# team-ergo-unipi/ergo_uvo

Measured on AMD Instinct MI355X. Metric: stereo frame-pairs/sec (detect+match+pose) @1920x1080, 3k kpts, higher is better.
Workload: dtype f32+f64

## Files before the change

ergo_uvo_amd/__init__.py:

```python
from __future__ import annotations

import collections
import ctypes as C

import numpy as np

from . import _lib

__all__ = ["Params", "Context", "StereoResult", "MonoResult", "UvoError", "KP_DTYPE", "DM_DTYPE", "build"]

build = _lib.build

KP_DTYPE = np.dtype([("x", "f4"), ("y", "f4"), ("size", "f4"), ("angle", "f4"), ("response", "f4"),
                     ("octave", "i4"), ("class_id", "i4")])
DM_DTYPE = np.dtype([("queryIdx", "i4"), ("trainIdx", "i4"), ("imgIdx", "i4"), ("distance", "f4")])

MEM_HOST, MEM_DEVICE = 0, 1
_STATUS = {1: "UVO_INVALID_ARG", 2: "UVO_TOO_FEW_POINTS", 3: "UVO_CAPACITY", 4: "UVO_HIP_ERROR", 5: "UVO_NO_DEVICE"}
_UVO_CAPACITY = 3


class UvoError(RuntimeError):
    def __init__(self, status: int, msg: str):
        super().__init__(f"{_STATUS.get(status, status)}: {msg}")
# ... 101 lines not shown
    def close(self):
        if getattr(self, "_h", None):
            self._lib.uvo_ctx_destroy(self._h)
            self._h = None

    def __del__(self):
        try:
            self.close()
        except Exception:
            pass

    @property
    def stream(self) -> int:
        return self._lib.uvo_ctx_stream(self._h)

    @property
    def warning(self) -> str:
        return (self._lib.uvo_ctx_warning(self._h) or b"").decode()

    def host_policy(self) -> dict:
        out = {}
        for kv in (self._lib.uvo_ctx_host_policy(self._h) or b"").decode().split():
            k, _, v = kv.partition("=")
            out[k] = float(v) if k == "cpu_budget" else (int(v) if k == "depth" else v)
        return out

    def set_producer_stream(self, stream):
        self._producer = stream
        if stream is None:
            self._check(self._lib.uvo_ctx_set_producer_stream(self._h, None, 0))
        elif stream != "torch":
            self._check(self._lib.uvo_ctx_set_producer_stream(self._h, C.c_void_p(int(getattr(stream, "cuda_stream", stream)) or None), 1))

    def _order_after_producer(self, *arrays):
        if self._producer == "torch" and any(_is_device(a) for a in arrays):
            import torch
            self._check(self._lib.uvo_ctx_set_producer_stream(self._h, C.c_void_p(torch.cuda.current_stream().cuda_stream or None), 1))

    def set_feature_detector(self, name: str):
        if name in ("AKAZE", "ORB"):
            self._check(self._lib.uvo_ctx_set_loop_detector(self._h, name.encode()))
            self._feature_akaze, self._feature_orb, self._feature_sift = name == "AKAZE", name == "ORB", False
            return
        self._check(self._lib.uvo_ctx_set_feature_detector(self._h, name.encode()))
        self._feature_sift = name == "SIFT"
        self._feature_akaze = self._feature_orb = False

# ... 473 lines not shown
```

ergo_uvo_amd/_lib.py:

```python
from __future__ import annotations

import ctypes as C
import os
import subprocess

_HERE = os.path.dirname(os.path.abspath(__file__))
CSRC = os.path.join(_HERE, "csrc")
LIB_PATH = os.environ.get("UVO_HIP_LIB") or os.path.join(_HERE, "lib", "libuvo_hip.so")

EXPORTS = [
    "uvo_params_default_stereo", "uvo_params_default_mono", "uvo_ctx_create", "uvo_ctx_destroy", "uvo_last_error",
    "uvo_ctx_stream", "uvo_ctx_set_params", "uvo_ctx_set_feature_detector", "uvo_ctx_set_loop_detector", "uvo_ctx_set_pnp_method", "uvo_ctx_set_producer_stream", "uvo_ctx_warning", "uvo_ctx_pending", "uvo_ctx_host_policy", "uvo_surf_detect", "uvo_sift_detect", "uvo_sift_layer", "uvo_akaze_detect", "uvo_akaze_plane", "uvo_orb_configure", "uvo_orb_set_pattern", "uvo_orb_detect", "uvo_orb_plane", "uvo_integral", "uvo_hessian_layer",
    "uvo_match_knn2_ratio", "uvo_match_knn2", "uvo_match_knn2_ratio_dim", "uvo_match_knn2_dim", "uvo_match_knn2_ratio_hamming", "uvo_match_knn2_hamming", "uvo_match_loop_knn2", "uvo_triangulate_points", "uvo_extract_3d_points",
    "uvo_solve_pnp_ransac", "uvo_reproject_errors", "uvo_rodrigues", "uvo_stereo_set_rig", "uvo_stereo_reset", "uvo_stereo_step",
    "uvo_stereo_set_depth", "uvo_stereo_submit", "uvo_stereo_collect",
    "uvo_stereo_get", "uvo_find_essential_mat", "uvo_recover_pose", "uvo_find_homography", "uvo_decompose_homography_mat",
    "uvo_recover_pose_homography", "uvo_select_estimation_method", "uvo_estimate_relative_pose", "uvo_mono_set_camera",
    "uvo_mono_reset", "uvo_mono_step", "uvo_mono_submit", "uvo_mono_collect", "uvo_mono_get", "uvo_get_image", "uvo_decode_image", "uvo_bayer_bggr2bgr", "uvo_resize_camera_matrix", "uvo_timing_enable", "uvo_timing_count", "uvo_timing_name", "uvo_timing_get", "uvo_timing_reset", "uvo_trace_enable", "uvo_trace_read",
]


EXPERIMENTAL = ["uvo_stereo_set_batch"]


def build(force: bool = False) -> str:
    srcs = [os.path.join(CSRC, f) for f in os.listdir(CSRC) if f.endswith((".hip", ".h"))]
    srcs.append(os.path.join(_HERE, "..", "include", "uvo_hip.h"))
    stale = not os.path.exists(LIB_PATH) or any(os.path.getmtime(s) > os.path.getmtime(LIB_PATH) for s in srcs)
    if force or stale:
        subprocess.check_call(["make", "-C", CSRC, "-s", "-j4"])
    return LIB_PATH


_lib = None


def lib() -> C.CDLL:
    global _lib
    if _lib is None:
        if not os.path.exists(LIB_PATH):
            build()
        try:
            import torch
        except ImportError:
            pass
# ... 3 lines not shown
        _lib.uvo_ctx_stream.restype = C.c_void_p
        _lib.uvo_ctx_stream.argtypes = [C.c_void_p]
        _lib.uvo_ctx_warning.restype = C.c_char_p
        _lib.uvo_ctx_warning.argtypes = [C.c_void_p]
        _lib.uvo_ctx_host_policy.restype = C.c_char_p
        _lib.uvo_ctx_host_policy.argtypes = [C.c_void_p]
        _lib.uvo_ctx_set_producer_stream.argtypes = [C.c_void_p, C.c_void_p, C.c_int]
        _lib.uvo_decode_image.argtypes = [C.c_void_p, C.c_void_p, C.c_size_t, C.c_char_p, C.c_void_p, C.c_size_t, C.c_int, C.c_void_p, C.c_void_p, C.c_void_p]
        _lib.uvo_sift_detect.argtypes = [C.c_void_p, C.c_void_p, C.c_int, C.c_int, C.c_int, C.c_int, C.c_int, C.c_int, C.c_double, C.c_double, C.c_double, C.c_void_p, C.c_void_p, C.c_int, C.c_void_p]
        _lib.uvo_ctx_set_feature_detector.argtypes = [C.c_void_p, C.c_char_p]
        _lib.uvo_ctx_set_loop_detector.argtypes = [C.c_void_p, C.c_char_p]
        _lib.uvo_ctx_set_pnp_method.argtypes = [C.c_void_p, C.c_int]
        _lib.uvo_match_loop_knn2.argtypes = [C.c_void_p, C.c_void_p, C.c_int, C.c_void_p, C.c_int, C.c_int, C.c_int, C.c_void_p, C.c_void_p]
        _lib.uvo_ctx_pending.restype = C.c_int
        _lib.uvo_ctx_pending.argtypes = [C.c_void_p]
        _lib.uvo_ctx_destroy.argtypes = [C.c_void_p]
        _lib.uvo_ctx_destroy.restype = None
        _lib.uvo_timing_name.restype = C.c_char_p
        _lib.uvo_timing_name.argtypes = [C.c_void_p, C.c_int]
        _lib.uvo_trace_read.restype = C.c_int
        _lib.uvo_trace_read.argtypes = [C.c_void_p, C.c_void_p, C.c_int]
        _lib.uvo_trace_enable.argtypes = [C.c_void_p, C.c_int]
        for name in EXPORTS + EXPERIMENTAL:
            getattr(_lib, name)
    return _lib
```

ergo_uvo_amd/csrc/ctx.hip:

```cpp
#include "uvo_ctx.h"
#include <pthread.h>
#include "uvo_epnp.h"
#include <string.h>
#include <sched.h>
#include <atomic>
#include <math.h>
#include <float.h>
#include <new>
#include <algorithm>
#include <atomic>
namespace uvo { extern bool g_bdbg; extern std::atomic<double> g_bstat[16]; double now_us(); void operator+=(std::atomic<double>& a, double v); }

using namespace uvo;

struct uvo_ctx : public uvo::Ctx {};

namespace {
uvo_status abi_caught(uvo_ctx* c) noexcept
{
    uvo_status st = UVO_HIP_ERROR;
    const char* what = "unexpected C++ exception inside libuvo_hip";
    static thread_local char text[160];
    try { throw; }
    catch (const std::bad_alloc&) { st = UVO_CAPACITY; what = "out of host memory (std::bad_alloc) inside libuvo_hip"; }
// ... 46 lines not shown

static void lane_worker(uvo_ctx* L);
__global__ void k_prime(int* sink, int n);
static void run_stage_b(uvo_ctx* L, bool stage_a_ok);
static uvo_status prime_lanes(uvo_ctx* c, int w, int h);
extern "C" uvo_status uvo_mono_collect(uvo_ctx* c, double dt, uvo_mono_result* out);
static void run_mono_stage_b(uvo_ctx* L, bool stage_a_ok);
static void destroy_one(uvo_ctx* c);
static uvo_status queue_stage_a(uvo_ctx* c, uvo_ctx* A, uvo_ctx* B);
struct GatherPair;
static hipError_t trace_alloc(Ctx* c)
{
    if (c->trace.empty()) {
        c->trace.resize(Ctx::kTraceRing);
        for (auto& r : c->trace) for (int k = 0; k < 8; k++) { hipError_t e = hipEventCreate(&r.ev[k]); if (e != hipSuccess) return e; }
    }
    c->trace_on = true;
    return hipSuccess;
}

namespace {
std::mutex g_pool_mu;
hipStream_t g_pool[64][2][uvo::Ctx::kMaxDepth];
bool pool_on() { static const bool on = !(getenv("UVO_STREAM_POOL") && atoi(getenv("UVO_STREAM_POOL")) == 0); return on; }
hipError_t stream_acquire(int device, int role, int lane, hipStream_t* out)
{
    if (pool_on() && lane >= 0 && lane < uvo::Ctx::kMaxDepth) {
        std::lock_guard<std::mutex> lk(g_pool_mu);
        hipStream_t& slot = g_pool[device & 63][role][lane];
        if (slot) { *out = slot; slot = nullptr; return hipSuccess; }
    }
    return hipStreamCreateWithFlags(out, hipStreamNonBlocking);
}
void stream_release(int device, int role, int lane, hipStream_t s)
{
    if (!s) return;
    (void)hipStreamSynchronize(s);
    if (pool_on() && lane >= 0 && lane < uvo::Ctx::kMaxDepth) {
        std::lock_guard<std::mutex> lk(g_pool_mu);
        hipStream_t& slot = g_pool[device & 63][role][lane];
        if (!slot) { slot = s; return; }
    }
    (void)hipStreamDestroy(s);
}
}

static const char* unsupported_params(const uvo_params* p)
{
    if (p->ITERATIONS_COUNT > 0 && p->PNP_METHOD_FLAG != 1)
        return "PNP_METHOD_FLAG: uvo_params takes only 1 (cv::SOLVEPNP_EPNP, the value shipped in stereo_VO_parameters.yaml); 2 (P3P), 3 (DLS) and 4 (UPNP) "
               "are set with uvo_ctx_set_pnp_method, 0 (ITERATIVE), 5 (AP3P) and above are not implemented";
    if (p->USE_EXTRINSIC_GUESS != 0) return "USE_EXTRINSIC_GUESS: only false is implemented (EPnP ignores the guess)";
    return nullptr;
}

static thread_local const char* t_create_refusal = nullptr;

static uvo_status create_one(const uvo_params* p, int device, int max_w, int max_h, int max_kpts, uvo_ctx** out, int lane = 0)
{
    if (!out) return UVO_INVALID_ARG;
    *out = nullptr;
    t_create_refusal = p ? unsupported_params(p) : nullptr;
    if (!p || max_w < 16 || max_h < 16 || max_kpts < 16 || t_create_refusal) return UVO_INVALID_ARG;
    int ndev = 0;
    if (hipGetDeviceCount(&ndev) != hipSuccess || ndev <= 0 || device < 0 || device >= ndev) return UVO_NO_DEVICE;
    if (hipSetDevice(device) != hipSuccess) return UVO_HIP_ERROR;
    uvo_ctx* c = new (std::nothrow) uvo_ctx();
    if (!c) return UVO_HIP_ERROR;
    c->p = *p; c->device = device; c->max_w = max_w; c->max_h = max_h; c->cap = max_kpts; c->lane_id = lane;
    const size_t cap = (size_t)max_kpts;
    const size_t npx = (size_t)max_w * max_h, nsum = (size_t)(max_w + 1) * (max_h + 1);
    const int nstrip = (max_h + 7) / 8;
    c->colpart_stride = ((max_w + 1 + 2047) / 2048) * 2048;
    const size_t nchunks = (cap + 127) / 128;
    hipError_t e = hipSuccess;
#define A(expr) do { if (e == hipSuccess) e = (expr); } while (0)
    A(stream_acquire(device, 0, lane, &c->stream));
    A(hipEventCreate(&c->ev0)); A(hipEventCreate(&c->ev1));
    c->plane_pw = ((max_w + 1 + 3) / 4 + 1 + 1) & ~1;
    c->plane_stride = c->plane_pw * ((max_h + 1 + 3) / 4 + 1);
    for (int i = 0; i < 2; i++) {
        A(dalloc(&c->d_planes[i], (size_t)16 * c->plane_stride));
        if (e == hipSuccess) e = hipMemset(c->d_planes[i], 0, sizeof(int32_t) * 16 * c->plane_stride);
        A(dalloc(&c->d_img[i], npx)); A(dalloc(&c->d_sum_base[i], nsum + 2 * kSumPad));
        if (e == hipSuccess) { e = hipMemset(c->d_sum_base[i], 0, sizeof(int32_t) * (nsum + 2 * kSumPad)); c->d_sum[i] = c->d_sum_base[i] + kSumPad; }
        A(dalloc(&c->d_cand[i], cap)); A(dalloc(&c->det[i].kps, cap)); A(dalloc(&c->det[i].desc, cap * 128));
        A(dalloc(&c->d_tmp_desc[i], cap * 128)); A(dalloc(&c->d_matches[i], cap));
        A(dalloc(&c->d_as_kpsL[i], cap)); A(dalloc(&c->d_as_kpsR[i], cap)); A(dalloc(&c->d_as_descL[i], cap * 128));
        A(dalloc(&c->d_as_pts4[i], cap)); A(dalloc(&c->d_as_cam1[i], cap * 3)); A(dalloc(&c->d_as_flag[i], cap));
    }
    c->surv_cap = 4 * (int)cap; A(dalloc(&c->d_surv, (size_t)c->surv_cap));
    A(dalloc(&c->d_colpart, (size_t)2 * nstrip * c->colpart_stride));
    A(dalloc(&c->d_DW, 400)); A(dalloc(&c->d_rank, cap * 2)); A(dalloc(&c->d_big_par, cap * 4)); A(dalloc(&c->d_big_patch, cap * 2 * 448));
    A(dalloc(&c->d_mpart, 2 * nchunks * cap)); A(dalloc(&c->d_mscratch, 2 * (nchunks + 4))); A(dalloc(&c->d_knn_idx, 2 * cap * 2)); A(dalloc(&c->d_knn_dist, 2 * cap * 2));
    A(dalloc(&c->d_x1, cap)); A(dalloc(&c->d_x2, cap)); A(dalloc(&c->d_xc, cap)); A(dalloc(&c->d_pts4, cap));
    A(dalloc(&c->d_cam1, cap * 3)); A(dalloc(&c->d_flag, cap)); A(dalloc(&c->d_tmp_idx, cap)); A(dalloc(&c->d_tmp_row, cap));
    if (const char* ww = getenv("UVO_WORKER_WAIT")) c->worker_wait = !strcmp(ww, "spin") ? 0 : (!strcmp(ww, "block-all") ? 2 : ((!strcmp(ww, "sleep") || !strcmp(ww, "block")) ? 3 : 1));
    c->wait_eff.store(c->worker_wait == 0 ? 0 : (c->worker_wait == 2 ? 2 : 1), std::memory_order_relaxed);
    A(hipEventCreateWithFlags(&c->evBlock, hipEventDisableTiming | hipEventBlockingSync));
    A(hipEventCreateWithFlags(&c->evPoll, hipEventDisableTiming));
    A(hipEventCreateWithFlags(&c->evB, hipEventDisableTiming | (c->worker_wait == 2 ? hipEventBlockingSync : 0)));
    for (int i = 0; i < 2; i++) {
        A(dalloc(&c->d_good_pts[i], cap * 3)); A(dalloc(&c->d_good_idx[i], cap));
        A(dalloc(&c->d_opts[i], cap * 3)); A(dalloc(&c->d_ipts[i], cap));
        A(hipEventCreateWithFlags(&c->evA[i], hipEventDisableTiming | ((i == 0 && c->worker_wait == 2) ? hipEventBlockingSync : 0)));
        A(hipHostMalloc(reinterpret_cast<void**>(&c->h_countsA[i]), sizeof(int) * CN_TOTAL));
    }
    A(hipEventCreateWithFlags(&c->evAS, hipEventDisableTiming));
    A(hipEventCreateWithFlags(&c->evSync, hipEventDisableTiming));
    A(hipEventCreateWithFlags(&c->evProducer, hipEventDisableTiming));
    A(hipEventCreateWithFlags(&c->evDet, hipEventDisableTiming)); A(hipEventCreateWithFlags(&c->evPrevRead, hipEventDisableTiming));
    {
        int least = 0, greatest = 0;
        const char* pe = getenv("UVO_PNP_PRIORITY");
        if (pe && atoi(pe) != 0 && hipDeviceGetStreamPriorityRange(&least, &greatest) == hipSuccess && greatest != least)
            A(hipStreamCreateWithPriority(&c->pnp_stream, hipStreamNonBlocking, greatest));
        else
            A(stream_acquire(device, 1, lane, &c->pnp_stream));
    }
    A(dalloc(&c->d_countsB, (size_t)4)); A(hipHostMalloc(reinterpret_cast<void**>(&c->h_countsB), sizeof(int) * 4));
    A(dalloc(&c->d_counts, (size_t)CN_TOTAL));
    A(dalloc(&c->d_subsets, (size_t)kMaxHyp * 5)); A(dalloc(&c->d_models, (size_t)kMaxHyp * 6)); A(dalloc(&c->d_hcount, (size_t)kMaxHyp));
    A(dalloc(&c->d_inliers, cap)); A(dalloc(&c->d_refit, cap * 21)); A(dalloc(&c->d_pose, (size_t)6));
    A(hipHostMalloc(reinterpret_cast<void**>(&c->h_counts), sizeof(int) * CN_TOTAL));
    A(hipHostMalloc(reinterpret_cast<void**>(&c->h_subsets), sizeof(int) * kMaxHyp * 5));
    A(hipHostMalloc(reinterpret_cast<void**>(&c->h_hcount), sizeof(int) * kMaxHyp));
    A(hipHostMalloc(reinterpret_cast<void**>(&c->h_pose), sizeof(double) * 6));
    A(dalloc(&c->d_rng_raw, (size_t)1024)); A(hipMalloc(&c->d_spec, 64)); A(hipHostMalloc(&c->h_spec, 64));
#undef A
    if (e != hipSuccess) { destroy_one(c); return UVO_HIP_ERROR; }
    c->d_cand_n = c->d_counts + CN_CAND0;
    c->det[0].n = c->d_counts + CN_NL; c->det[1].n = c->d_counts + CN_NR;
    c->d_nmatch = c->d_counts + CN_M;
    c->d_as_n = c->d_counts + CN_AS0;
    c->d_big_n = c->d_counts + CN_BIG0;
    if (surf_build_area_tables(c) != UVO_OK) { destroy_one(c); return UVO_HIP_ERROR; }
    {
        std::vector<unsigned> raw(1024);
        uint64_t state = (uint64_t)-1;
        for (auto& v : raw) v = rng_next(state);
        if (hipMemcpy(c->d_rng_raw, raw.data(), sizeof(unsigned) * raw.size(), hipMemcpyHostToDevice) != hipSuccess ||
// ... 48 lines not shown
        double q = -1, per = 0;
        if (FILE* g = fopen("/sys/fs/cgroup/cpu/cpu.cfs_quota_us", "r")) { if (fscanf(g, "%lf", &q) != 1) q = -1; fclose(g); }
        if (FILE* g = fopen("/sys/fs/cgroup/cpu/cpu.cfs_period_us", "r")) { if (fscanf(g, "%lf", &per) != 1) per = 0; fclose(g); }
        if (q > 0 && per > 0) b = std::min(b, q / per);
    }
    if (const char* e = getenv("UVO_CPU_BUDGET")) { const double v = atof(e); if (v > 0) b = std::min(b, v); }
    return b;
}
static void apply_wait_policy(uvo_ctx* c)
{
    const int depth = (int)c->lanes.size();
    c->cpu_budget = host_cpu_budget();
    int eff = c->worker_wait == 0 ? 0 : (c->worker_wait == 2 ? 2 : 1);
    if (c->worker_wait == 1 && c->cpu_budget >= 2.0 * (depth + 2)) eff = 0;
    for (Ctx* l : c->lanes) l->wait_eff.store(eff, std::memory_order_release);
    if (const char* e = getenv("UVO_STAGE_B")) c->stage_b_mode = !strcmp(e, "device") ? 1 : (!strcmp(e, "worker") ? 0 : -1);
}
static bool stage_b_on_device(const uvo_ctx* c)
{
    if (c->stage_b_mode >= 0) return c->stage_b_mode == 1;
    return c->cpu_budget < (double)c->lanes.size() + 3.0;
}

static uvo_status set_depth(uvo_ctx* c, int depth)
{
    if (depth < 1 || depth > Ctx::kMaxDepth) { c->err = "pipeline depth must be 1..16"; return UVO_INVALID_ARG; }
    if (c->n_pending != 0) { c->err = "pipeline depth cannot change while pairs are in flight"; return UVO_INVALID_ARG; }
    while ((int)c->lanes.size() > depth) { destroy_one(static_cast<uvo_ctx*>(c->lanes.back())); c->lanes.pop_back(); }
    while ((int)c->lanes.size() < depth) {
        uvo_ctx* l = nullptr;
        uvo_status st = create_one(&c->p, c->device, c->max_w, c->max_h, c->cap, &l, (int)c->lanes.size());
        if (st != UVO_OK) { c->err = "could not allocate a further pipeline lane"; return st; }
        l->master = c; l->lane_id = (int)c->lanes.size(); l->timing = c->timing;
        if (c->trace_on && !l->trace_on && trace_alloc(l) != hipSuccess) { destroy_one(l); c->err = "could not allocate a further pipeline lane"; return UVO_HIP_ERROR; }
        c->lanes.push_back(l);
    }
    apply_wait_policy(c);
    c->warning.clear();
    {
        const char* q = getenv("GPU_MAX_HW_QUEUES");
        const int nq = q ? atoi(q) : 4;
        if (depth > 2 && nq < 2 * depth)
            c->warning = "GPU_MAX_HW_QUEUES = " + std::to_string(nq) + " with " + std::to_string(depth) + " pipeline lanes (two HIP streams each): lanes share "
                         "hardware queues and the pipeline runs well below its rate; set GPU_MAX_HW_QUEUES >= " + std::to_string(2 * depth) + " before the HIP runtime starts";
    }
    if (c->primed_w > 0) UVO_TRY(prime_lanes(c, c->primed_w, c->primed_h));
    if (c->prev_lane >= depth || c->next_lane >= depth) { c->vo_initialized = false; c->init_matches.clear(); c->prev_lane = 0; c->next_lane = 0; c->prev_sync = true; }
    return UVO_OK;
}

static void precreate_streams(int device)
{
    static const int order = getenv("UVO_STREAM_ORDER") ? atoi(getenv("UVO_STREAM_ORDER")) : 0;
    if (order < 1 || order > 2 || !pool_on()) return;
    const int depth = getenv("UVO_PIPELINE_DEPTH") ? std::min((int)uvo::Ctx::kMaxDepth, std::max(1, atoi(getenv("UVO_PIPELINE_DEPTH")))) : 6;
    if (hipSetDevice(device) != hipSuccess) return;
    std::lock_guard<std::mutex> lk(g_pool_mu);
    int* sink = nullptr;
    if (hipMalloc(reinterpret_cast<void**>(&sink), 64) != hipSuccess) return;
    for (int pass = 0; pass < 2; pass++) {
        const int role = order == 1 ? pass : 1 - pass;
        for (int l = 0; l < depth; l++) {
            hipStream_t& slot = g_pool[device & 63][role][l];
            if (slot) continue;
            if (hipStreamCreateWithFlags(&slot, hipStreamNonBlocking) != hipSuccess) { slot = nullptr; continue; }
            hipLaunchKernelGGL(k_prime, dim3(1), dim3(64), 0, slot, sink, 1);
            (void)hipStreamSynchronize(slot);
        }
    }
    (void)hipFree(sink);
}

extern "C" uvo_status uvo_ctx_create(const uvo_params* p, int device, int max_w, int max_h, int max_kpts, uvo_ctx** out)
try {
    precreate_streams(device);
    uvo_status st = create_one(p, device, max_w, max_h, max_kpts, out);
    if (st != UVO_OK) return st;
    (*out)->lanes.push_back(*out);
    if (getenv("UVO_MAX_B")) (*out)->max_b = std::min(16, std::max(1, atoi(getenv("UVO_MAX_B"))));
    if (getenv("UVO_A_OVERLAP")) (*out)->a_overlap = std::min(16, std::max(0, atoi(getenv("UVO_A_OVERLAP"))));
    if (getenv("UVO_MAX_B_MONO")) (*out)->max_b_mono = std::min(16, std::max(1, atoi(getenv("UVO_MAX_B_MONO"))));
    if (getenv("UVO_A_OVERLAP2")) (*out)->a_overlap2 = std::min(4, std::max(0, atoi(getenv("UVO_A_OVERLAP2"))));
    if (getenv("UVO_BATCH")) (*out)->batch = atoi(getenv("UVO_BATCH")) == 2 ? 2 : 1;
    if (getenv("UVO_A_OVERLAP_MONO")) (*out)->a_overlap_mono = std::min(8, std::max(0, atoi(getenv("UVO_A_OVERLAP_MONO"))));
    st = set_depth(*out, 2);
    if (st != UVO_OK) { uvo_ctx_destroy(*out); *out = nullptr; }
    return st;
} UVO_ABI_CATCH(nullptr)

extern "C" uvo_status uvo_stereo_set_batch(uvo_ctx* c, int pairs)
try {
    if (!c) return UVO_INVALID_ARG;
    if (pairs != 1 && pairs != 2) { c->err = "uvo_stereo_set_batch: 1 or 2 pairs per launch set"; return UVO_INVALID_ARG; }
    if (c->n_pending != 0) { c->err = "the launch mode cannot change while pairs are in flight"; return UVO_INVALID_ARG; }
    c->batch = pairs;
    return UVO_OK;
} UVO_ABI_CATCH(c)

// ... 33 lines not shown
    }
    if (c->stream) (void)hipStreamSynchronize(c->stream);
    for (int i = 0; i < 2; i++) {
        (void)hipFree(c->d_img[i]); (void)hipFree(c->d_sum_base[i]); (void)hipFree(c->d_planes[i]); (void)hipFree(c->d_cand[i]); (void)hipFree(c->det[i].kps);
        (void)hipFree(c->det[i].desc); (void)hipFree(c->d_tmp_desc[i]); (void)hipFree(c->d_matches[i]);
        (void)hipFree(c->d_as_kpsL[i]); (void)hipFree(c->d_as_kpsR[i]); (void)hipFree(c->d_as_descL[i]);
        (void)hipFree(c->d_as_pts4[i]); (void)hipFree(c->d_as_cam1[i]); (void)hipFree(c->d_as_flag[i]);
    }
    if (c->pnp_stream) (void)hipStreamSynchronize(c->pnp_stream);
    mono_ws_free(c);
    pre_ws_free(c);
    codec_ws_free(c);
    sift_ws_free(c);
    akaze_ws_free(c);
    orb_ws_free(c);
    void* ptrs[] = { c->d_hess_order, c->d_surv, c->d_octpat, c->d_colpart, c->d_DW, c->d_rank, c->d_big_par, c->d_big_patch, c->d_area_tabs, c->d_area_iscale, c->d_ori_w, c->d_mpart, c->d_mscratch, c->d_knn_idx, c->d_knn_dist, c->d_x1, c->d_x2, c->d_xc, c->d_pts4, c->d_cam1,
                     c->d_flag, c->d_tmp_idx, c->d_tmp_row, c->d_good_pts[0], c->d_good_pts[1], c->d_good_idx[0], c->d_good_idx[1], c->d_opts[0], c->d_opts[1],
                     c->d_ipts[0], c->d_ipts[1], c->d_counts, c->d_countsB, c->d_subsets, c->d_models,
                     c->d_hcount, c->d_inliers, c->d_refit, c->d_pose };
    for (void* p : ptrs) (void)hipFree(p);
    (void)hipHostFree(c->h_counts); (void)hipHostFree(c->h_subsets); (void)hipHostFree(c->h_hcount); (void)hipHostFree(c->h_pose);
    (void)hipHostFree(c->h_countsB); (void)hipHostFree(c->h_spec); (void)hipFree(c->d_rng_raw); (void)hipFree(c->d_spec);
    for (int i = 0; i < 2; i++) { (void)hipHostFree(c->h_countsA[i]); if (c->evA[i]) (void)hipEventDestroy(c->evA[i]); }
    {
        const char* pe = getenv("UVO_PNP_PRIORITY");
        if (c->pnp_stream && pe && atoi(pe) != 0) (void)hipStreamDestroy(c->pnp_stream);
        else stream_release(c->device, 1, c->lane_id, c->pnp_stream);
    }
    if (c->evAS) (void)hipEventDestroy(c->evAS);
    if (c->evBlock) (void)hipEventDestroy(c->evBlock);
    if (c->evPoll) (void)hipEventDestroy(c->evPoll);
    if (c->evB) (void)hipEventDestroy(c->evB);
    if (c->evSync) (void)hipEventDestroy(c->evSync);
    if (c->evProducer) (void)hipEventDestroy(c->evProducer);
    for (auto& r : c->trace) for (int k = 0; k < 8; k++) if (r.ev[k]) (void)hipEventDestroy(r.ev[k]);
    if (c->evDet) (void)hipEventDestroy(c->evDet);
    if (c->evPrevRead) (void)hipEventDestroy(c->evPrevRead);
    if (c->ev0) (void)hipEventDestroy(c->ev0);
    if (c->ev1) (void)hipEventDestroy(c->ev1);
    stream_release(c->device, 0, c->lane_id, c->stream);
    delete c;
}

extern "C" const char* uvo_last_error(const uvo_ctx* c) { return c ? c->err.c_str() : (t_create_refusal ? t_create_refusal : "null context"); }
extern "C" void* uvo_ctx_stream(uvo_ctx* c) { return c ? (void*)c->stream : nullptr; }
extern "C" uvo_status uvo_ctx_set_params(uvo_ctx* c, const uvo_params* p)
try {
    if (!c || !p) return UVO_INVALID_ARG;
    if (c->n_pending != 0) { c->err = "parameters cannot change while pairs are in flight"; return UVO_INVALID_ARG; }
    if (const char* why = unsupported_params(p)) { c->err = why; return UVO_INVALID_ARG; }
    if ((p->SURF_EXTENDED != 0) != (c->p.SURF_EXTENDED != 0) && (c->vo_initialized || c->mono_initialized)) {
        c->err = "SURF_EXTENDED changes the descriptor width: the previous frame's descriptors held by the running VO loop would not match (uvo_stereo_reset / uvo_mono_reset first)";
        return UVO_INVALID_ARG;
    }
    for (Ctx* l : c->lanes) l->p = *p;
    return UVO_OK;
} UVO_ABI_CATCH(c)
extern "C" uvo_status uvo_ctx_set_producer_stream(uvo_ctx* c, void* hip_stream, int enabled)
try {
    if (!c) return UVO_INVALID_ARG;
    c->producer_stream = static_cast<hipStream_t>(hip_stream); c->has_producer = enabled != 0;
    return UVO_OK;
} UVO_ABI_CATCH(c)
extern "C" const char* uvo_ctx_warning(const uvo_ctx* c) { return c ? c->warning.c_str() : ""; }
extern "C" int uvo_ctx_pending(const uvo_ctx* c) { return c ? c->n_pending : 0; }
extern "C" const char* uvo_ctx_host_policy(uvo_ctx* c)
try {
    if (!c) return "";
    static const char* const wn[3] = { "poll", "timed-sleep+poll", "interrupt" };
    char buf[160];
    snprintf(buf, sizeof(buf), "wait=%s stage_b=%s cpu_budget=%.2f depth=%d", wn[c->wait_eff.load() % 3], stage_b_on_device(c) ? "device" : "worker",
             c->cpu_budget > 1e8 ? -1.0 : c->cpu_budget, (int)c->lanes.size());
    c->policy_text = buf;
    return c->policy_text.c_str();
} UVO_ABI_CATCH_RET(c, "")

static uvo_status wait_for_producer(uvo_ctx* m, Ctx* L, int mem)
{
    if (mem != UVO_MEM_DEVICE || !m->has_producer) return UVO_OK;
    UVO_HIP_TRY(m, hipEventRecord(L->evProducer, m->producer_stream));
    UVO_HIP_TRY(m, hipStreamWaitEvent(L->stream, L->evProducer, 0));
    return UVO_OK;
}
static uvo_status need_idle(uvo_ctx* c, const char* who)
{
    if (c->n_pending == 0) return UVO_OK;
    c->err = std::string(who) + ": collect the pairs / frames in flight first (the operator uses lane 0's buffers)";
    return UVO_INVALID_ARG;
}

static uvo_status fail(uvo_ctx* c, uvo_status s, const char* msg) { c->err = msg; return s; }

namespace uvo {
static inline void poll_pause() { for (int i = 0; i < 40; i++) __builtin_ia32_pause(); }
hipError_t poll_event(hipEvent_t ev)
// ... 643 lines not shown
    const int depth = (int)c->lanes.size();
    if (c->n_pending >= depth) return fail(c, UVO_INVALID_ARG, "uvo_stereo_submit: the pipeline is full; collect a pair first (uvo_stereo_set_depth)");
    if (c->timing && c->n_pending > 0) return fail(c, UVO_INVALID_ARG, "timing mode measures one pair at a time: collect before submitting");
    (void)hipSetDevice(c->device);
    const uvo_params& p = c->p;
    if (!c->vo_initialized) {
        uvo_stereo_result res;
        memset(&res, 0, sizeof(res));
        UVO_TRY(wait_for_producer(c, c, mem));
        UVO_TRY(surf_upload(c, 0, left, w, h, stride, mem));
        UVO_TRY(surf_upload(c, 1, right, w, h, stride, mem));
        UVO_TRY(detect_dispatch(c, 2));
        UVO_TRY(stereo_init_step(c, &res));
        UVO_TRY(prime_lanes(c, w, h));
        UVO_TRY(prepare_lane_detectors(c, w, h, 2));
        c->stereo_init_results.push_back(res);
        c->inflight[c->n_pending++] = Ctx::kInflightStereoInit; c->n_submitted++;
        c->next_lane = 0;
        return UVO_OK;
    }
    const int li = c->next_lane;
    Range r_submit("uvo:stereo_submit");
    uvo_ctx* L = static_cast<uvo_ctx*>(c->lanes[li]);
    L->pending = Ctx::Pending();
    L->pending.used = true;
    Ctx::StagePlan& pl = L->plan;
    pl.lane = li; pl.prev_lane = c->prev_lane; pl.prev_buf = c->prev_buf; pl.prev_sync = c->prev_sync; pl.curr = L->as_w;
    pl.pending_before = c->n_pending; pl.trace_slot = -1;
    if (L->trace_on) {
        L->trace_cur = (int)(L->trace_count++ % Ctx::kTraceRing);
        pl.trace_slot = L->trace_cur;
        Ctx::TraceRec* tr = &L->trace[L->trace_cur];
        tr->pair = c->n_submitted; tr->b_used = false; tr->det_marked = false;
        for (double& v : tr->host_us) v = 0;
        tr->host_us[0] = uvo::now_us();
    }
    const bool may_batch = c->batch == 2 && depth >= 2 && !c->in_sync_step && !c->timing && c->loop_detector() == 0 && p.SURF_UPRIGHT && p.SURF_OCTAVES_NUMBER == 4;
    uvo_ctx* S = c->stashed_lane >= 0 ? static_cast<uvo_ctx*>(c->lanes[c->stashed_lane]) : nullptr;
    hipStream_t own = L->stream;
    if (S && may_batch) L->stream = S->stream;
    uvo_status up = wait_for_producer(c, L, mem);
    if (up == UVO_OK) up = surf_upload(L, 0, left, w, h, stride, mem);
    if (up == UVO_OK) up = surf_upload(L, 1, right, w, h, stride, mem);
    L->stream = own;
    if (up != UVO_OK) { if (L != c) c->err = L->err; L->pending.used = false; return up; }
    L->as_w = pl.curr ^ 1;
// ... 186 lines not shown
static void lane_worker(uvo_ctx* L)
{
    { char nm[16]; snprintf(nm, sizeof(nm), "uvo-lane%d", L->lane_id); (void)pthread_setname_np(pthread_self(), nm); }
    (void)hipSetDevice(L->device);
    std::unique_lock<std::mutex> lk(L->mu);
    for (;;) {
        if (L->job.state != 1 && !L->quit) { lk.unlock(); poll_job_state(L, 1, 2000.0); lk.lock(); }
        L->cv.wait(lk, [&] { return L->quit || L->job.state == 1; });
        if (L->quit) return;
        lk.unlock();
        const double t0 = g_bdbg ? now_us() : 0;
        const bool stage_a_ok = wait_stage_a(L);
        if (g_bdbg) g_bstat[0] += now_us() - t0;
        Ctx::TraceRec* wtr = (L->trace_on && L->trace_cur >= 0 && L->job.kind == 0) ? &L->trace[L->trace_cur] : nullptr;
        if (wtr) wtr->host_us[3] = now_us();
        {
            Ctx* m = L->master ? L->master : L;
            std::unique_lock<std::mutex> g(m->b_mu);
            const double tw = g_bdbg ? now_us() : 0;
            const int limit = L->job.kind == 1 ? m->max_b_mono : m->max_b;
            m->b_cv.wait(g, [&] { return m->b_running < limit; });
            if (g_bdbg) g_bstat[5] += now_us() - tw;
            m->b_running++;
            g.unlock();
            if (wtr) wtr->host_us[4] = now_us();
            try {
                if (L->job.kind == 1) { const double tb = g_bdbg ? now_us() : 0; run_mono_stage_b(L, stage_a_ok); if (g_bdbg) { g_bstat[1] += now_us() - tb; g_bstat[4] += 1; } }
                else if (L->job.kind == 2) { hipLaunchKernelGGL(k_prime, dim3(1), dim3(64), 0, L->pnp_stream, L->d_countsB, 1); (void)host_sync(L, L->pnp_stream); }
                else run_stage_b(L, stage_a_ok);
            } catch (...) {
                L->job.st = abi_caught(L); L->job.ran = 0;
                try { L->job.err = L->err; } catch (...) { L->job.err.clear(); }
            }
            if (wtr) wtr->host_us[5] = now_us();
            g.lock();
            m->b_running--;
            m->b_cv.notify_one();
        }
        lk.lock();
        L->job.state = 2;
        L->job_state_a.store(2, std::memory_order_release);
        L->cv.notify_all();
    }
}

extern "C" uvo_status uvo_stereo_collect(uvo_ctx* c, double dt, uvo_stereo_result* out)
try {
    if (!c || !out) return UVO_INVALID_ARG;
    if (c->n_pending <= 0) return fail(c, UVO_INVALID_ARG, "uvo_stereo_collect: nothing submitted");
    if (c->inflight[0] == Ctx::kInflightMonoInit || (c->inflight[0] >= 0 && c->lanes[c->inflight[0]]->job.kind != 0))
        return fail(c, UVO_INVALID_ARG, "uvo_stereo_collect: the oldest entry in flight is a mono frame (uvo_mono_collect)");
    (void)hipSetDevice(c->device);
    Range r_collect("uvo:stereo_collect");
    const uvo_params& p = c->p;
    const int li = c->inflight[0];
    for (int i = 1; i < c->n_pending; i++) c->inflight[i - 1] = c->inflight[i];
    c->n_pending--; c->n_collected++;
    if (li == Ctx::kInflightStereoInit) {
// ... 499 lines not shown
    if (c->mono_matched) {
        if (c->use_binary()) UVO_TRY(match_knn2_bin(c, BIN_L2, reinterpret_cast<const uint8_t*>(c->d_as_descL[0]), nullptr, c->mono_n_prev,
                                                    reinterpret_cast<const uint8_t*>(c->det[0].desc), c->det[0].n, c->cap));
        else UVO_TRY(match_knn2(c, c->d_as_descL[0], nullptr, c->mono_n_prev, c->det[0].desc, c->det[0].n, c->cap));
        UVO_TRY(match_ratio_compact(c, nullptr, c->mono_n_prev, (float)p.LOWE_RATIO_THRESHOLD, c->d_matches[0], c->d_nmatch, c->cap));
        hipLaunchKernelGGL(k_gather_mono_pairs, dim3((c->cap + 255) / 256), dim3(256), 0, c->stream, c->d_matches[0], c->d_counts + CN_M, c->cap,
                           c->d_as_kpsL[0], c->det[0].kps, c->d_x1, c->d_x2);
        UVO_HIP_TRY(c, hipGetLastError());
        UVO_TRY(mono_prep_launch(c, c->stream, c->mono_K, p.DISTANCE));
    }
    UVO_HIP_TRY(c, hipMemcpyAsync(c->h_countsA[0], c->d_counts, sizeof(int) * CN_TOTAL, hipMemcpyDeviceToHost, c->stream));
    UVO_HIP_TRY(c, host_sync(c, c->stream));
    memcpy(c->h_counts, c->h_countsA[0], sizeof(int) * CN_TOTAL);
    UVO_TRY(check_cand_overflow(c, 1));
    const int n = c->h_counts[CN_NL];
    out->n_kps = n;
    c->kp_hint = n;
    c->mono_dev_n = n;
    auto roll_state = [&]() -> uvo_status {
        if (n) {
            UVO_HIP_TRY(c, hipMemcpyAsync(c->d_as_descL[0], c->det[0].desc, sizeof(float) * c->loop_words() * (size_t)n, hipMemcpyDeviceToDevice, c->stream));
            UVO_HIP_TRY(c, hipMemcpyAsync(c->d_as_kpsL[0], c->det[0].kps, sizeof(uvo_keypoint) * (size_t)n, hipMemcpyDeviceToDevice, c->stream));
        }
        c->mono_n_prev = n;
        return UVO_OK;
    };
    if (!c->mono_initialized) {
        UVO_TRY(roll_state());
        if (n >= p.MIN_NUM_FEATURES) c->mono_initialized = true;
        return UVO_OK;
    }
    c->job.kind = 1; c->job.range = range;
    run_mono_stage_b(c, true);
    if (c->job.st != UVO_OK) { const uvo_status st_ = c->job.st; c->err = c->job.err; return st_; }
    apply_mono_result(c, c->job, dt, out);
    return roll_state();
} UVO_ABI_CATCH(c)

extern "C" uvo_status uvo_mono_submit(uvo_ctx* c, const uint8_t* img, int w, int h, int stride, int mem, double range)
try {
    if (!c || !img) return UVO_INVALID_ARG;
    if (!c->mono_cam_set) return fail(c, UVO_INVALID_ARG, "uvo_mono_set_camera has not been called");
    const int depth = (int)c->lanes.size();
    if (depth < 2) return fail(c, UVO_INVALID_ARG, "uvo_mono_submit needs at least two lanes (uvo_stereo_set_depth): a frame is matched against the previous lane's buffers");
    UVO_TRY(need_loop_table(c));
    if (c->n_pending >= depth) return fail(c, UVO_INVALID_ARG, "uvo_mono_submit: the pipeline is full; collect a frame first (uvo_stereo_set_depth)");
    (void)hipSetDevice(c->device);
    Range r_submit("uvo:mono_submit");
    const uvo_params& p = c->p;
    if (!c->mono_initialized) {
        uvo_mono_result r;
        memset(&r, 0, sizeof(r));
        UVO_TRY(uvo_mono_step(c, img, w, h, stride, mem, range, 1.0, &r));
        c->mono_init_results.push_back(r);
        c->inflight[c->n_pending++] = Ctx::kInflightMonoInit; c->n_submitted++;
        c->prev_lane = 0; c->next_lane = 1 % depth;
        UVO_HIP_TRY(c, hipEventRecord(c->evDet, c->stream));
        UVO_TRY(prime_lanes(c, w, h));
        UVO_TRY(prepare_lane_detectors(c, w, h, 1));
        return UVO_OK;
    }
    const int li = c->next_lane;
    uvo_ctx* L = static_cast<uvo_ctx*>(c->lanes[li]);
    Ctx* P = c->lanes[c->prev_lane];
    c->mono_pipelined = true;
#define LANE_TRY(expr) do { uvo_status st_ = (expr); if (st_ != UVO_OK) { if (L != c) c->err = L->err; return st_; } } while (0)
    hipStream_t st = L->stream;
    L->pending = Ctx::Pending(); L->pending.used = true;
    if (L->prev_read_pending) { UVO_HIP_TRY(c, hipStreamWaitEvent(st, L->evPrevRead, 0)); L->prev_read_pending = false; }
    UVO_TRY(wait_for_producer(c, L, mem));
    LANE_TRY(surf_upload(L, 0, img, w, h, stride, mem));
    if (c->a_overlap_mono > 0 && depth > c->a_overlap_mono) {
        Ctx* H = c->lanes[(li + depth - c->a_overlap_mono) % depth];
        if (c->n_pending >= c->a_overlap_mono) (void)uvo::poll_event(H->evA[1]);
    }
    LANE_TRY(detect_dispatch(L, 1));
    UVO_HIP_TRY(c, hipEventRecord(L->evDet, st));
    int* cn = L->d_counts;
    const int cap = c->cap;
    if (P != L) UVO_HIP_TRY(c, hipStreamWaitEvent(st, P->evDet, 0));
    if (L->use_binary()) LANE_TRY(match_knn2_bin(L, BIN_L2, reinterpret_cast<const uint8_t*>(P->det[0].desc), P->det[0].n, cap,
                                                 reinterpret_cast<const uint8_t*>(L->det[0].desc), L->det[0].n, cap));
    else LANE_TRY(match_knn2(L, P->det[0].desc, P->det[0].n, cap, L->det[0].desc, L->det[0].n, cap));
    LANE_TRY(match_ratio_compact(L, P->det[0].n, cap, (float)p.LOWE_RATIO_THRESHOLD, L->d_matches[0], cn + CN_M, cap));
    hipLaunchKernelGGL(k_gather_mono_pairs, dim3((cap + 255) / 256), dim3(256), 0, st, L->d_matches[0], cn + CN_M, cap,
                       P->det[0].kps, L->det[0].kps, L->d_x1, L->d_x2);
    UVO_HIP_TRY(c, hipGetLastError());
    LANE_TRY(mono_prep_launch(L, st, c->mono_K, p.DISTANCE));
// ... 135 lines not shown
```

ergo_uvo_amd/csrc/uvo_ctx.h:

```cpp
#pragma once
#include <hip/hip_runtime.h>
#include <string>
#include <thread>
#include <mutex>
#include <condition_variable>
#include <atomic>
#include <vector>
#include <deque>
#include <stdint.h>
#include "../../include/uvo_hip.h"
#include "uvo_experimental.h"

namespace uvo {

#define UVO_HIP_TRY(c, expr)                                                                  \
    do {                                                                                      \
        hipError_t _e = (expr);                                                               \
        if (_e != hipSuccess) {                                                               \
            (c)->err = std::string(#expr) + ": " + hipGetErrorString(_e);                     \
            return UVO_HIP_ERROR;                                                             \
        }                                                                                     \
    } while (0)

#define UVO_TRY(expr)                                                                         \
// ... 81 lines not shown
    double* d_cam1 = nullptr;
    int* d_flag = nullptr;
    double* d_good_pts[2] = {nullptr, nullptr};  int* d_good_idx[2] = {nullptr, nullptr};
    float* d_opts[2] = {nullptr, nullptr};  uvo_point2f* d_ipts[2] = {nullptr, nullptr};
    int* d_tmp_idx = nullptr;
    int* d_tmp_row = nullptr;
    int* d_counts = nullptr;
    int* h_counts = nullptr;

    int* d_subsets = nullptr;
    int* h_subsets = nullptr;
    double* d_models = nullptr;
    int* d_hcount = nullptr;  int* h_hcount = nullptr;
    int* d_inliers = nullptr;
    double* d_refit = nullptr;
    double* d_pose = nullptr;  double* h_pose = nullptr;
    unsigned* d_rng_raw = nullptr;
    void* d_spec = nullptr; void* h_spec = nullptr;
    bool spec_queued = false;
    hipEvent_t evSync = nullptr; bool inline_b = false;
    bool in_sync_step = false;

    hipStream_t pnp_stream = nullptr;
    int* d_countsB = nullptr;  int* h_countsB = nullptr;
    hipEvent_t evA[2] = {nullptr, nullptr};
    int worker_wait = 1;
    std::atomic<int> wait_eff{1};
    int stage_b_mode = -1;
    bool dev_b = false;
    hipEvent_t evB = nullptr;
    double cpu_budget = 0;
    double stage_a_mean_us = 0;
    double t_handover_us = 0;
    std::atomic<int> job_state_a{0};
    hipEvent_t evBlock = nullptr;
    hipEvent_t evPoll = nullptr;
    int* h_countsA[2] = {nullptr, nullptr};
    hipEvent_t evAS = nullptr;
    int a_overlap = 2;
    int a_overlap_mono = 4;
    int batch = 1;
    int a_overlap2 = 2;
    struct StagePlan { int lane = -1, prev_lane = 0, prev_buf = 0, curr = 0, pending_before = 0; bool prev_sync = true; int trace_slot = -1; };
    StagePlan plan;
    int stashed_lane = -1;
    std::vector<Ctx*> lanes;
// ... 181 lines not shown
```

ergo_uvo_amd/csrc/uvo_experimental.h:

```cpp
#pragma once
#include "../../include/uvo_hip.h"
#ifdef __cplusplus
extern "C" {
#endif
uvo_status uvo_stereo_set_batch(uvo_ctx* c, int pairs);
#ifdef __cplusplus
}
#endif
```

Measured before the change: 3135.

## Share a small set of role-based streams across pipeline lanes when hardware queues are scarce

When GPU_MAX_HW_QUEUES is below twice the pipeline depth, lanes no longer each use their own two streams. Stage-A work round-robins over a few shared streams and PnP (stage B) picks the least-loaded shared stream, so the number of streams stays within the hardware queue budget and pairs stop oversubscribing queues. This removes the eager stream pre-creation path and adds a stream-creation counter. The risk is extra serialization on the shared streams, plus added synchronization when a lane switches streams.

```diff
diff --git a/ergo_uvo_amd/__init__.py b/ergo_uvo_amd/__init__.py
--- a/ergo_uvo_amd/__init__.py
+++ b/ergo_uvo_amd/__init__.py
@@ -147,7 +147,7 @@
         out = {}
         for kv in (self._lib.uvo_ctx_host_policy(self._h) or b"").decode().split():
             k, _, v = kv.partition("=")
-            out[k] = float(v) if k == "cpu_budget" else (int(v) if k == "depth" else v)
+            out[k] = float(v) if k == "cpu_budget" else (int(v) if k in ("depth", "hw_queues", "a_streams", "b_streams") else v)
         return out
 
     def set_producer_stream(self, stream):
diff --git a/ergo_uvo_amd/_lib.py b/ergo_uvo_amd/_lib.py
--- a/ergo_uvo_amd/_lib.py
+++ b/ergo_uvo_amd/_lib.py
@@ -20,7 +20,7 @@
 ]
 
 
-EXPERIMENTAL = ["uvo_stereo_set_batch"]
+EXPERIMENTAL = ["uvo_stereo_set_batch", "uvo_streams_created"]
 
 
 def build(force: bool = False) -> str:
@@ -70,5 +70,7 @@
         _lib.uvo_trace_read.argtypes = [C.c_void_p, C.c_void_p, C.c_int]
         _lib.uvo_trace_enable.argtypes = [C.c_void_p, C.c_int]
         for name in EXPORTS + EXPERIMENTAL:
+            if name == "uvo_streams_created" and os.environ.get("UVO_HIP_LIB"):
+                continue
             getattr(_lib, name)
     return _lib
diff --git a/ergo_uvo_amd/csrc/ctx.hip b/ergo_uvo_amd/csrc/ctx.hip
--- a/ergo_uvo_amd/csrc/ctx.hip
+++ b/ergo_uvo_amd/csrc/ctx.hip
@@ -92,6 +92,7 @@
 namespace {
 std::mutex g_pool_mu;
 hipStream_t g_pool[64][2][uvo::Ctx::kMaxDepth];
+std::atomic<int> g_streams_created{0};
 bool pool_on() { static const bool on = !(getenv("UVO_STREAM_POOL") && atoi(getenv("UVO_STREAM_POOL")) == 0); return on; }
 hipError_t stream_acquire(int device, int role, int lane, hipStream_t* out)
 {
@@ -100,6 +101,7 @@
         hipStream_t& slot = g_pool[device & 63][role][lane];
         if (slot) { *out = slot; slot = nullptr; return hipSuccess; }
     }
+    g_streams_created.fetch_add(1, std::memory_order_relaxed);
     return hipStreamCreateWithFlags(out, hipStreamNonBlocking);
 }
 void stream_release(int device, int role, int lane, hipStream_t s)
@@ -114,6 +116,10 @@
     (void)hipStreamDestroy(s);
 }
 }
+extern "C" int uvo_streams_created(void)
+try {
+    return g_streams_created.load(std::memory_order_relaxed);
+} UVO_ABI_CATCH_RET(nullptr, 0)
 
 static const char* unsupported_params(const uvo_params* p)
 {
@@ -145,7 +151,7 @@
     const size_t nchunks = (cap + 127) / 128;
     hipError_t e = hipSuccess;
 #define A(expr) do { if (e == hipSuccess) e = (expr); } while (0)
-    A(stream_acquire(device, 0, lane, &c->stream));
+    A(stream_acquire(device, 0, lane, &c->stream)); c->own_stream = c->stream;
     A(hipEventCreate(&c->ev0)); A(hipEventCreate(&c->ev1));
     c->plane_pw = ((max_w + 1 + 3) / 4 + 1 + 1) & ~1;
     c->plane_stride = c->plane_pw * ((max_h + 1 + 3) / 4 + 1);
@@ -183,10 +189,12 @@
     {
         int least = 0, greatest = 0;
         const char* pe = getenv("UVO_PNP_PRIORITY");
-        if (pe && atoi(pe) != 0 && hipDeviceGetStreamPriorityRange(&least, &greatest) == hipSuccess && greatest != least)
+        if (pe && atoi(pe) != 0 && hipDeviceGetStreamPriorityRange(&least, &greatest) == hipSuccess && greatest != least) {
             A(hipStreamCreateWithPriority(&c->pnp_stream, hipStreamNonBlocking, greatest));
-        else
+            c->own_pnp_priority = true;
+        } else
             A(stream_acquire(device, 1, lane, &c->pnp_stream));
+        c->own_pnp_stream = c->pnp_stream;
     }
     A(dalloc(&c->d_countsB, (size_t)4)); A(hipHostMalloc(reinterpret_cast<void**>(&c->h_countsB), sizeof(int) * 4));
     A(dalloc(&c->d_counts, (size_t)CN_TOTAL));
@@ -281,10 +289,36 @@
     return c->cpu_budget < (double)c->lanes.size() + 3.0;
 }
 
+static int hw_queue_budget() { const char* q = getenv("GPU_MAX_HW_QUEUES"); const int nq = q ? atoi(q) : 4; return nq > 0 ? nq : 4; }
+static int forced_stream_plan()
+{
+    static const int f = [] { const char* e = getenv("UVO_STREAM_PLAN"); return !e ? 0 : (!strcmp(e, "lanes") ? 1 : (!strcmp(e, "shared") ? 2 : 0)); }();
+    return f;
+}
+static bool roles_in_use(const uvo_ctx* c) { return c->plan_shared && !stage_b_on_device(c); }
+static uvo_status lane_take_streams(uvo_ctx* c, uvo_ctx* L, bool roles)
+{
+    hipStream_t a = roles ? c->sh_a[c->n_submitted % c->n_a] : L->own_stream;
+    if (L->tail_unsynced && a != L->stream) UVO_HIP_TRY(c, hipStreamSynchronize(L->stream));
+    L->tail_unsynced = false;
+    L->stream = a; L->pnp_stream = roles ? c->sh_b[c->n_submitted % c->n_b] : L->own_pnp_stream;
+    L->on_roles = roles;
+    return UVO_OK;
+}
+
 static uvo_status set_depth(uvo_ctx* c, int depth)
 {
     if (depth < 1 || depth > Ctx::kMaxDepth) { c->err = "pipeline depth must be 1..16"; return UVO_INVALID_ARG; }
     if (c->n_pending != 0) { c->err = "pipeline depth cannot change while pairs are in flight"; return UVO_INVALID_ARG; }
+    const int Q = hw_queue_budget();
+    const bool shared = forced_stream_plan() == 2 || (forced_stream_plan() == 0 && Q < 2 * depth);
+    int n_a = depth, n_b = depth;
+    if (shared) {
+        const int want_a = c->a_overlap > 0 ? std::min(c->a_overlap, depth) : depth;
+        n_a = std::max(1, std::min(want_a, Q - 1));
+        n_b = std::max(1, std::min(std::min(c->max_b, depth), Q - n_a));
+    }
+    const bool plan_changed = shared != c->plan_shared || (shared && n_b != c->n_b);
     while ((int)c->lanes.size() > depth) { destroy_one(static_cast<uvo_ctx*>(c->lanes.back())); c->lanes.pop_back(); }
     while ((int)c->lanes.size() < depth) {
         uvo_ctx* l = nullptr;
@@ -294,45 +328,30 @@
         if (c->trace_on && !l->trace_on && trace_alloc(l) != hipSuccess) { destroy_one(l); c->err = "could not allocate a further pipeline lane"; return UVO_HIP_ERROR; }
         c->lanes.push_back(l);
     }
+    for (Ctx* l : c->lanes) { l->stream = l->own_stream; l->pnp_stream = l->own_pnp_stream; l->b_slot = -1; l->on_roles = false; }
+    for (int i = 0; i < Ctx::kMaxDepth; i++) {
+        c->sh_a[i] = (shared && i < n_a) ? c->lanes[i]->own_stream : nullptr;
+        c->sh_b[i] = (shared && i < n_b) ? c->lanes[i]->own_pnp_stream : nullptr;
+    }
+    { std::lock_guard<std::mutex> g(c->b_mu); for (int& v : c->b_load) v = 0; }
+    c->plan_shared = shared; c->hw_queues = Q; c->n_a = n_a; c->n_b = n_b;
     apply_wait_policy(c);
     c->warning.clear();
-    {
-        const char* q = getenv("GPU_MAX_HW_QUEUES");
-        const int nq = q ? atoi(q) : 4;
-        if (depth > 2 && nq < 2 * depth)
-            c->warning = "GPU_MAX_HW_QUEUES = " + std::to_string(nq) + " with " + std::to_string(depth) + " pipeline lanes (two HIP streams each): lanes share "
-                         "hardware queues and the pipeline runs well below its rate; set GPU_MAX_HW_QUEUES >= " + std::to_string(2 * depth) + " before the HIP runtime starts";
-    }
-    if (c->primed_w > 0) UVO_TRY(prime_lanes(c, c->primed_w, c->primed_h));
+    if (depth > 2 && Q < 2 * depth && !roles_in_use(c))
+        c->warning = "GPU_MAX_HW_QUEUES = " + std::to_string(Q) + " with " + std::to_string(depth) + " pipeline lanes (two HIP streams each): lanes share "
+                     "hardware queues and the pipeline runs well below its rate; set GPU_MAX_HW_QUEUES >= " + std::to_string(2 * depth) + " before the HIP runtime starts";
+    else if (shared && depth > 1 && Q < 3)
+        c->warning = "GPU_MAX_HW_QUEUES = " + std::to_string(Q) + ": the pipeline needs three hardware queues (two stage-A streams and a PnP stream) to keep "
+                     "one pair's detection out from behind another pair's PnP kernels; set GPU_MAX_HW_QUEUES >= 3 before the HIP runtime starts";
+    const int primed_w = c->primed_w, primed_h = c->primed_h;
+    if (plan_changed) for (Ctx* l : c->lanes) l->primed_w = l->primed_h = 0;
+    if (primed_w > 0) UVO_TRY(prime_lanes(c, primed_w, primed_h));
     if (c->prev_lane >= depth || c->next_lane >= depth) { c->vo_initialized = false; c->init_matches.clear(); c->prev_lane = 0; c->next_lane = 0; c->prev_sync = true; }
     return UVO_OK;
 }
 
-static void precreate_streams(int device)
-{
-    static const int order = getenv("UVO_STREAM_ORDER") ? atoi(getenv("UVO_STREAM_ORDER")) : 0;
-    if (order < 1 || order > 2 || !pool_on()) return;
-    const int depth = getenv("UVO_PIPELINE_DEPTH") ? std::min((int)uvo::Ctx::kMaxDepth, std::max(1, atoi(getenv("UVO_PIPELINE_DEPTH")))) : 6;
-    if (hipSetDevice(device) != hipSuccess) return;
-    std::lock_guard<std::mutex> lk(g_pool_mu);
-    int* sink = nullptr;
-    if (hipMalloc(reinterpret_cast<void**>(&sink), 64) != hipSuccess) return;
-    for (int pass = 0; pass < 2; pass++) {
-        const int role = order == 1 ? pass : 1 - pass;
-        for (int l = 0; l < depth; l++) {
-            hipStream_t& slot = g_pool[device & 63][role][l];
-            if (slot) continue;
-            if (hipStreamCreateWithFlags(&slot, hipStreamNonBlocking) != hipSuccess) { slot = nullptr; continue; }
-            hipLaunchKernelGGL(k_prime, dim3(1), dim3(64), 0, slot, sink, 1);
-            (void)hipStreamSynchronize(slot);
-        }
-    }
-    (void)hipFree(sink);
-}
-
 extern "C" uvo_status uvo_ctx_create(const uvo_params* p, int device, int max_w, int max_h, int max_kpts, uvo_ctx** out)
 try {
-    precreate_streams(device);
     uvo_status st = create_one(p, device, max_w, max_h, max_kpts, out);
     if (st != UVO_OK) return st;
     (*out)->lanes.push_back(*out);
@@ -412,11 +431,8 @@
     (void)hipHostFree(c->h_counts); (void)hipHostFree(c->h_subsets); (void)hipHostFree(c->h_hcount); (void)hipHostFree(c->h_pose);
     (void)hipHostFree(c->h_countsB); (void)hipHostFree(c->h_spec); (void)hipFree(c->d_rng_raw); (void)hipFree(c->d_spec);
     for (int i = 0; i < 2; i++) { (void)hipHostFree(c->h_countsA[i]); if (c->evA[i]) (void)hipEventDestroy(c->evA[i]); }
-    {
-        const char* pe = getenv("UVO_PNP_PRIORITY");
-        if (c->pnp_stream && pe && atoi(pe) != 0) (void)hipStreamDestroy(c->pnp_stream);
-        else stream_release(c->device, 1, c->lane_id, c->pnp_stream);
-    }
+    if (c->own_pnp_stream && c->own_pnp_priority) { (void)hipStreamSynchronize(c->own_pnp_stream); (void)hipStreamDestroy(c->own_pnp_stream); }
+    else stream_release(c->device, 1, c->lane_id, c->own_pnp_stream);
     if (c->evAS) (void)hipEventDestroy(c->evAS);
     if (c->evBlock) (void)hipEventDestroy(c->evBlock);
     if (c->evPoll) (void)hipEventDestroy(c->evPoll);
@@ -428,7 +444,7 @@
     if (c->evPrevRead) (void)hipEventDestroy(c->evPrevRead);
     if (c->ev0) (void)hipEventDestroy(c->ev0);
     if (c->ev1) (void)hipEventDestroy(c->ev1);
-    stream_release(c->device, 0, c->lane_id, c->stream);
+    stream_release(c->device, 0, c->lane_id, c->own_stream);
     delete c;
 }
 
@@ -458,9 +474,10 @@
 try {
     if (!c) return "";
     static const char* const wn[3] = { "poll", "timed-sleep+poll", "interrupt" };
-    char buf[160];
-    snprintf(buf, sizeof(buf), "wait=%s stage_b=%s cpu_budget=%.2f depth=%d", wn[c->wait_eff.load() % 3], stage_b_on_device(c) ? "device" : "worker",
-             c->cpu_budget > 1e8 ? -1.0 : c->cpu_budget, (int)c->lanes.size());
+    char buf[224];
+    snprintf(buf, sizeof(buf), "wait=%s stage_b=%s cpu_budget=%.2f depth=%d hw_queues=%d a_streams=%d b_streams=%d", wn[c->wait_eff.load() % 3],
+             stage_b_on_device(c) ? "device" : "worker", c->cpu_budget > 1e8 ? -1.0 : c->cpu_budget, (int)c->lanes.size(), c->hw_queues,
+             roles_in_use(c) ? c->n_a : (int)c->lanes.size(), roles_in_use(c) ? c->n_b : (int)c->lanes.size());
     c->policy_text = buf;
     return c->policy_text.c_str();
 } UVO_ABI_CATCH_RET(c, "")
@@ -1150,6 +1167,7 @@
     const int li = c->next_lane;
     Range r_submit("uvo:stereo_submit");
     uvo_ctx* L = static_cast<uvo_ctx*>(c->lanes[li]);
+    UVO_TRY(lane_take_streams(c, L, roles_in_use(c) && !c->in_sync_step));
     L->pending = Ctx::Pending();
     L->pending.used = true;
     Ctx::StagePlan& pl = L->plan;
@@ -1382,11 +1400,20 @@
             m->b_cv.wait(g, [&] { return m->b_running < limit; });
             if (g_bdbg) g_bstat[5] += now_us() - tw;
             m->b_running++;
+            if (L->job.kind == 0 && m->plan_shared && L->on_roles) {
+                int best = 0;
+                for (int i = 1; i < m->n_b; i++) if (m->b_load[i] < m->b_load[best]) best = i;
+                m->b_load[best]++; L->b_slot = best; L->pnp_stream = m->sh_b[best];
+            }
             g.unlock();
             if (wtr) wtr->host_us[4] = now_us();
             try {
                 if (L->job.kind == 1) { const double tb = g_bdbg ? now_us() : 0; run_mono_stage_b(L, stage_a_ok); if (g_bdbg) { g_bstat[1] += now_us() - tb; g_bstat[4] += 1; } }
-                else if (L->job.kind == 2) { hipLaunchKernelGGL(k_prime, dim3(1), dim3(64), 0, L->pnp_stream, L->d_countsB, 1); (void)host_sync(L, L->pnp_stream); }
+                else if (L->job.kind == 2) {
+                    hipLaunchKernelGGL(k_prime, dim3(1), dim3(64), 0, L->pnp_stream, L->d_countsB, 1); (void)host_sync(L, L->pnp_stream);
+                    for (int i = 0; i < m->n_b && m->plan_shared; i++)
+                        if (m->sh_b[i] && m->sh_b[i] != L->pnp_stream) { hipLaunchKernelGGL(k_prime, dim3(1), dim3(64), 0, m->sh_b[i], L->d_countsB, 1); (void)host_sync(L, m->sh_b[i]); }
+                }
                 else run_stage_b(L, stage_a_ok);
             } catch (...) {
                 L->job.st = abi_caught(L); L->job.ran = 0;
@@ -1394,6 +1421,7 @@
             }
             if (wtr) wtr->host_us[5] = now_us();
             g.lock();
+            if (L->b_slot >= 0) { m->b_load[L->b_slot]--; L->b_slot = -1; }
             m->b_running--;
             m->b_cv.notify_one();
         }
@@ -1939,7 +1967,7 @@
             UVO_HIP_TRY(c, hipMemcpyAsync(c->d_as_descL[0], c->det[0].desc, sizeof(float) * c->loop_words() * (size_t)n, hipMemcpyDeviceToDevice, c->stream));
             UVO_HIP_TRY(c, hipMemcpyAsync(c->d_as_kpsL[0], c->det[0].kps, sizeof(uvo_keypoint) * (size_t)n, hipMemcpyDeviceToDevice, c->stream));
         }
-        c->mono_n_prev = n;
+        c->mono_n_prev = n; c->tail_unsynced = n > 0;
         return UVO_OK;
     };
     if (!c->mono_initialized) {
@@ -1981,6 +2009,7 @@
     uvo_ctx* L = static_cast<uvo_ctx*>(c->lanes[li]);
     Ctx* P = c->lanes[c->prev_lane];
     c->mono_pipelined = true;
+    UVO_TRY(lane_take_streams(c, L, false));
 #define LANE_TRY(expr) do { uvo_status st_ = (expr); if (st_ != UVO_OK) { if (L != c) c->err = L->err; return st_; } } while (0)
     hipStream_t st = L->stream;
     L->pending = Ctx::Pending(); L->pending.used = true;
diff --git a/ergo_uvo_amd/csrc/uvo_ctx.h b/ergo_uvo_amd/csrc/uvo_ctx.h
--- a/ergo_uvo_amd/csrc/uvo_ctx.h
+++ b/ergo_uvo_amd/csrc/uvo_ctx.h
@@ -127,6 +127,15 @@
     bool in_sync_step = false;
 
     hipStream_t pnp_stream = nullptr;
+    hipStream_t own_stream = nullptr, own_pnp_stream = nullptr;
+    bool own_pnp_priority = false;
+    bool plan_shared = false;
+    int hw_queues = 4, n_a = 1, n_b = 1;
+    hipStream_t sh_a[16] = {nullptr}, sh_b[16] = {nullptr};
+    int b_load[16] = {0};
+    int b_slot = -1;
+    bool on_roles = false;
+    bool tail_unsynced = false;
     int* d_countsB = nullptr;  int* h_countsB = nullptr;
     hipEvent_t evA[2] = {nullptr, nullptr};
     int worker_wait = 1;
diff --git a/ergo_uvo_amd/csrc/uvo_experimental.h b/ergo_uvo_amd/csrc/uvo_experimental.h
--- a/ergo_uvo_amd/csrc/uvo_experimental.h
+++ b/ergo_uvo_amd/csrc/uvo_experimental.h
@@ -4,6 +4,7 @@
 extern "C" {
 #endif
 uvo_status uvo_stereo_set_batch(uvo_ctx* c, int pairs);
+int uvo_streams_created(void);
 #ifdef __cplusplus
 }
 #endif
```

Result: faster. 3527 (median of 6 runs) (+12.5%).
